# SAIC-MONTREAL/multimodal-dynamics

Measured on AMD Instinct MI355X. Metric: visuotactile samples/sec (train) + ELBO vs CPU ref, cnn-mvae 64x64 bs256 @1/2/4/8 GPU, higher is better.
Workload: dtype f32x3; 1 GPU; cnn-mvae visuotactile+pose 64x64, bs=256 per GPU, fp32 storage and results, GEMMs in the fp32x3 arithmetic (exact three-term bf16 split of the fp32 operands, six of nine products on the bf16 matrix cores, fp32 accumulate; error vs fp64 <= native fp32 MFMA), seq_modeling train step (7 subset ELBOs + backward + Adam), BASELINE configs[1]; global_batch=256, parallelism=dp1, bn=local, launch=hip_graph

## Files before the change

include/mmdyn_hip.h:

```cpp
#ifndef MMDYN_HIP_H
#define MMDYN_HIP_H

#include <stdint.h>

#ifdef __cplusplus
extern "C" {
#endif

#define MMDYN_OK 0
#define MMDYN_ERR_SHAPE (-1)
#define MMDYN_ERR_NULL (-2)
#define MMDYN_ERR_RANGE (-3)

#define MMDYN_ACT_NONE 0
#define MMDYN_ACT_SWISH 1
#define MMDYN_ACT_RELU 2

#define MMDYN_DENSE 0
#define MMDYN_CONV 1
#define MMDYN_TCONV_S2P1 2
#define MMDYN_IM2COL3 3

#define MMDYN_TCONV_S1P0 4

// ... 16 lines not shown
int mmdyn_igemm_slab_floats(int mode, int G, int Bg, int Hi, int Wi, int Cin, int Ho, int Wo, int N);

int mmdyn_igemm_nt_bf16(const float* A, const float* Bp, const float* bias, float* C, float* C_act,
                        float* stats, float* ws, int mode, int G, int Bg, int Hi, int Wi, int Cin,
                        int Ho, int Wo, int N, int ldc, int stride, int offset, int act, int splitk,
                        void* stream);
int mmdyn_igemm_nt_f16(const float* A, const float* Bp, const float* bias, float* C, float* C_act,
                       float* stats, float* ws, int mode, int G, int Bg, int Hi, int Wi, int Cin,
                       int Ho, int Wo, int N, int ldc, int stride, int offset, int act, int splitk,
                       void* stream);
int mmdyn_igemm_stat_tiles(int mode, int G, int Bg, int Hi, int Wi, int Cin, int Ho, int Wo, int N);
int mmdyn_igemm_stat_tiles_bf16(int mode, int G, int Bg, int Hi, int Wi, int Cin, int Ho, int Wo, int N);
int mmdyn_igemm_stat_tiles_mx(int mode, int G, int Bg, int Hi, int Wi, int Cin, int Ho, int Wo, int N, int flags);
int mmdyn_igemm_slab_floats_mx(int mode, int G, int Bg, int Hi, int Wi, int Cin, int Ho, int Wo, int N, int flags);
int mmdyn_igemm_nt_grouped(const void* A, const void* Bp, const float* bias, void* C, void* C_act, const void* u, int G,
                           int rows, int K, int N, int act, int flags, void* stream);
int mmdyn_splitk_reduce(const float* ws, const float* bias, float* C, float* C_act, int splitk,
                        int rows, int N, int act, void* stream);

int mmdyn_wgrad_tn(const float* D, const float* Gt, float* partial, int mode, int Bt, int Hr, int Wr,
                   int Cd, int Hi, int Wi, int Cg, int stride, int offset, int chunks, void* stream);
int mmdyn_wgrad_tn_bf16(const float* D, const float* Gt, float* partial, int mode, int Bt, int Hr, int Wr,
                        int Cd, int Hi, int Wi, int Cg, int stride, int offset, int chunks, void* stream);
int mmdyn_wgrad_tn_f16(const float* D, const float* Gt, float* partial, int mode, int Bt, int Hr, int Wr,
                       int Cd, int Hi, int Wi, int Cg, int stride, int offset, int chunks, void* stream);
int mmdyn_wgrad_tn_grouped(const void* D, const void* Gt, float* partial, int G, int rows, int Cd, int Cg, int chunks,
                           int flags, void* stream);
int mmdyn_wgrad_out3_bn(const void* y, const float* mean, const float* rstd, const float* gamma, const float* beta,
                        const float* Gt, float* partial, int G, int Bg, int Hr, int chunks, int y_b16, void* stream);
int mmdyn_wgrad_chunks(int mode, int rows, int Cd, int Cg);
int mmdyn_wgrad_chunks_mx(int mode, int rows, int Cd, int Cg, int flags);
int mmdyn_wgrad_reduce(const float* partial, float* canon, int chunks, int taps, int Cd, int Cg,
                       int cg_canon, int perm, float beta, void* stream);

int mmdyn_pack_conv_weight(const float* Wc, float* P, int d0, int d1, int swap, void* stream);
int mmdyn_repack2d(const float* in, float* out, int rows_in, int cols_in, int rows_out, int cols_out,
                   int mode, void* stream);

int mmdyn_repack2d_ld(const float* in, float* out, int rows_in, int cols_in, int rows_out, int cols_out,
                      int ld_out, int mode, void* stream);
int mmdyn_pack_conv_weight_b16(const float* Wc, void* P, int d0, int d1, int swap, int half, void* stream);
int mmdyn_repack2d_ld_b16(const float* in, void* out, int rows_in, int cols_in, int rows_out, int cols_out,
                          int ld_out, int mode, int half, void* stream);
typedef struct {
  const float* src;
  float* dst;
  int kind, rows_in, cols_in, rows_out, cols_out, ld_out;
  int dst_bf16;
} mmdyn_pack_entry;
int mmdyn_pack_plan(const mmdyn_pack_entry* plan_dev, int n, void* stream);

int mmdyn_im2col_nchw3(const float* x, float* col, int Bt, int H, int W, void* stream);
int mmdyn_col2im_k4(const float* col, float* out, int Bt, int Hi, int Wi, int Ho, int Wo, int C,
                    int ldcol, int stride, int pad, int tap_major, void* stream);

int mmdyn_tconv_out3_fwd(const float* a, const float* w, float* out, int Bt, int Hi, int Wi, void* stream);
int mmdyn_tconv_out3_bn_fwd(const void* y, const float* mean, const float* rstd, const float* gamma, const float* beta,
                            const float* w, float* out, int G, int Bg, int Hi, int Wi, int b16, void* stream);
int mmdyn_tconv_out3_bn_bce(const void* y, const float* mean, const float* rstd, const float* gamma, const float* beta,
                            const float* w, float* logits, int logits_group, const float* target, const float* mask,
                            int mask_channels, float* dlogit, double* loss_slots, double* unmasked_slots,
                            const int* slot_of_group, float grad_scale, int G, int Bg, int Hi, int Wi, int b16, void* stream);
int mmdyn_tconv_out3_bn_bce_rows(const void* y, const float* mean, const float* rstd, const float* gamma, const float* beta,
                                 const float* w, float* logits, int logits_group, const float* target, const float* mask,
                                 int mask_channels, double* loss_rows, double* unmasked_rows, const int* slot_of_group,
                                 int n_slots, int G, int Bg, int Hi, int Wi, int b16, void* stream);
// ... 200 lines not shown
```

multimodal-dynamics_amd/csrc/wgrad_geom.h:

```cpp
#pragma once
#include "common.h"

struct WgradGeom {
  int d_b16, g_b16;
  int f16;
  int mode;
  int rows;
  int Hr, Wr, Cd;
  int Hi, Wi, Cg;
  int rs, ro;
  int ntaps, chunks, rows_per_chunk;
  int groups;
  int x3;
  int pre;
};

#ifdef MMDYN_LAB
int mmdyn_wgrad_ws_try(const float* D, const float* Gt, float* partial, const WgradGeom& g, hipStream_t st);
#else
static inline int mmdyn_wgrad_ws_try(const float*, const float*, float*, const WgradGeom&, hipStream_t) { return 1; }
#endif

int mmdyn_wgrad_p3_try(const void* D, const void* Gt, float* partial, const WgradGeom& g, int Bt, hipStream_t st);
int mmdyn_wgrad_p3_chunks(int rows, int Cd, int Cg);
```

multimodal-dynamics_amd/csrc/wgrad_tn.hip:

```cpp
#include <stdlib.h>
#include "common.h"
#include "wgrad_geom.h"

namespace {


constexpr int RK = 32;

typedef __bf16 bf16x4 __attribute__((ext_vector_type(4)));
typedef short s16x4 __attribute__((ext_vector_type(4)));
typedef _Float16 f16x4 __attribute__((ext_vector_type(4)));
__device__ __forceinline__ f16x4 pack4_f16(float a, float b, float c, float d) {
  f16x4 r;
  r[0] = (_Float16)a; r[1] = (_Float16)b; r[2] = (_Float16)c; r[3] = (_Float16)d;
  return r;
}
__device__ __forceinline__ s16x4 pack4_bf16(float a, float b, float c, float d) {
  bf16x4 r;
  r[0] = (__bf16)a; r[1] = (__bf16)b; r[2] = (__bf16)c; r[3] = (__bf16)d;
  return __builtin_bit_cast(s16x4, r);
}

template <int BX> struct x3_ld { static constexpr int v = (BX == 32) ? 32 : BX + 32; };
template <int MODE, int BD, int BG, int WD, int WG, int WK, bool BF16, int ST, bool X3 = false, int PRE = 0>
__global__ __launch_bounds__(256) void wgrad_tn_kernel(const float* __restrict__ D,
                                                       const float* __restrict__ Gt,
                                                       float* __restrict__ partial, const WgradGeom g) {
  static_assert(!X3 || (!BF16 && ST == 0 && WK == 1 && MODE != MMDYN_IM2COL3), "the three-term split is a variant of the fp32 kernel");
  static_assert(PRE == 0 || X3, "operands that arrive split belong to the three-term split arithmetic");
  constexpr bool PD = (PRE & 1) != 0, PG = (PRE & 2) != 0;
  constexpr int DT = WD / 32, GT = WG / 32;
  constexpr int WAVES_G = BG / WG;
  constexpr int WAVES_DG = (BD / WD) * WAVES_G;
  static_assert(WAVES_DG * WK == 4, "4 waves per block");
  constexpr int KPW = (RK / 2) / WK;
  constexpr int DV = BD / 4, GV = BG / 4;
  constexpr int D_LOADS = (RK * DV) / 256, G_LOADS = (RK * GV) / 256;
  static_assert(D_LOADS >= 1 && G_LOADS >= 1, "tile too small for 256 threads");

  extern __shared__ __attribute__((aligned(16))) char smem[];
  float* Ds = reinterpret_cast<float*>(smem);
  float* Gs = Ds + RK * BD;
  constexpr int LDD = x3_ld<BD>::v, LDG = x3_ld<BG>::v;
  bf16_t* Ds16 = reinterpret_cast<bf16_t*>(smem);
  bf16_t* Gs16 = Ds16 + 3 * RK * LDD;

  const int tid = threadIdx.x, lane = tid & 63, wave = tid >> 6;
  const int wk = wave / WAVES_DG, wdg = wave % WAVES_DG;
  const int wd = wdg / WAVES_G, wg = wdg % WAVES_G;
  const int tiles_g = g.Cg / BG;
  const int td = blockIdx.x / tiles_g, tg = blockIdx.x - td * tiles_g;
  const int cd0 = td * BD, cg0 = tg * BG;
  const int tap = blockIdx.y;
  const int ngrp = g.groups > 1 ? g.groups : 1;
  const int zb = gridDim.z / ngrp;
  const int grp = blockIdx.z / zb, chunk = blockIdx.z - grp * zb;
  const int dh = (MODE == MMDYN_CONV) ? (tap >> 2) : 0;
  const int dw = (MODE == MMDYN_CONV) ? (tap & 3) : 0;
  const int HWr = g.Hr * g.Wr;

  const int row_begin = grp * g.rows + chunk * g.rows_per_chunk;
  const int row_end = min((grp + 1) * g.rows, row_begin + g.rows_per_chunk);

  const float inv_hw = 1.0f / (float)HWr, inv_w = 1.0f / (float)g.Wr;
  auto fdiv = [](int n, int d, float inv, int& q, int& r) {
    q = (int)((float)n * inv);
    r = n - q * d;
    if (r < 0) { q -= 1; r += d; }
    if (r >= d) { q += 1; r -= d; }
  };
  f32x4 rd[D_LOADS], rg[G_LOADS];
  constexpr int DV8 = BD / 8, GV8 = BG / 8;
  constexpr int D_LOADS8 = (RK * DV8) / 256, G_LOADS8 = (RK * GV8) / 256;
  static_assert(PRE == 0 || (D_LOADS8 >= 1 && G_LOADS8 >= 1), "plane granules: tile too small for 256 threads");
  u32x4 pd[PD ? D_LOADS8 : 1][3], pg[PG ? G_LOADS8 : 1][3];
  unsigned okd = 0, okg = 0;
  auto gload = [&](int r0) {
    if constexpr (PD) {
#pragma unroll
      for (int i = 0; i < D_LOADS8; ++i) {
        const int idx = tid + 256 * i;
        const int r = idx / DV8, v = idx - r * DV8;
        const int row = r0 + r;
        const bool ok = row < row_end;
        const bf16_t* b = reinterpret_cast<const bf16_t*>(D) + (size_t)(ok ? row : 0) * 3 * g.Cd + cd0 + v * 8;
#pragma unroll
        for (int p = 0; p < 3; ++p) pd[i][p] = *reinterpret_cast<const u32x4*>(b + p * g.Cd);
        okd = ok ? (okd | (1u << i)) : (okd & ~(1u << i));
      }
    } else
#pragma unroll
    for (int i = 0; i < D_LOADS; ++i) {
      const int idx = tid + 256 * i;
      const int r = idx / DV, v = idx - r * DV;
      const int row = r0 + r;
// ... 120 lines not shown
          uint2 hh, mm, ll;
          split3_bf16(x[0], x[1], hh.x, mm.x, ll.x);
          split3_bf16(x[2], x[3], hh.y, mm.y, ll.y);
          *reinterpret_cast<uint2*>(&Gs16[o]) = hh;
          *reinterpret_cast<uint2*>(&Gs16[RK * LDG + o]) = mm;
          *reinterpret_cast<uint2*>(&Gs16[2 * RK * LDG + o]) = ll;
        }
      }
      return;
    }
#pragma unroll
    for (int i = 0; i < D_LOADS; ++i)
      reinterpret_cast<f32x4*>(Ds)[tid + 256 * i] = ((okd >> i) & 1u) ? rd[i] : zero;
#pragma unroll
    for (int i = 0; i < G_LOADS; ++i) {
      const unsigned m = okg >> (4 * i);
      f32x4 v;
      v[0] = (m & 1u) ? rg[i][0] : 0.f;
      v[1] = (m & 2u) ? rg[i][1] : 0.f;
      v[2] = (m & 4u) ? rg[i][2] : 0.f;
      v[3] = (m & 8u) ? rg[i][3] : 0.f;
      reinterpret_cast<f32x4*>(Gs)[tid + 256 * i] = v;
    }
  };

  f32x16 acc[DT][GT];
#pragma unroll
  for (int a = 0; a < DT; ++a)
#pragma unroll
    for (int b = 0; b < GT; ++b)
#pragma unroll
      for (int e = 0; e < 16; ++e) acc[a][b][e] = 0.f;

  const int h = lane >> 5, cl = lane & 31;
  if (row_begin < row_end) {
    gload(row_begin);
    lds_store();
    __syncthreads();
    for (int r0 = row_begin; r0 < row_end; r0 += RK) {
      gload(r0 + RK);
      __builtin_amdgcn_sched_barrier(0);
      if constexpr (X3) {
        const int gq = lane >> 4, tq = (lane >> 2) & 3, tp = lane & 3;
        const int trow = 8 * (gq >> 1) + tq, tcol = 16 * (gq & 1) + 4 * tp;
        typedef __attribute__((address_space(3))) s16x4* lds_s16x4_p;
        typedef __bf16 xb16x8 __attribute__((ext_vector_type(8)));
        auto frag = [&](const bf16_t* tile, int ld, int col0, int k0) {
          const s16x4 lo = __builtin_amdgcn_ds_read_tr16_b64_v4i16((lds_s16x4_p)(&tile[(k0 + trow) * ld + col0 + tcol]));
          const s16x4 hi = __builtin_amdgcn_ds_read_tr16_b64_v4i16((lds_s16x4_p)(&tile[(k0 + trow + 4) * ld + col0 + tcol]));
          typedef short s16x8 __attribute__((ext_vector_type(8)));
          const s16x8 v = {lo[0], lo[1], lo[2], lo[3], hi[0], hi[1], hi[2], hi[3]};
          return __builtin_bit_cast(xb16x8, v);
        };
#pragma unroll
        for (int kc = 0; kc < 2; ++kc) {
          xb16x8 pa[3][DT], pb[3][GT];
#pragma unroll
          for (int p = 0; p < 3; ++p) {
#pragma unroll
            for (int a = 0; a < DT; ++a) pa[p][a] = frag(Ds16 + p * RK * LDD, LDD, wd * WD + a * 32, kc * 16);
#pragma unroll
            for (int b = 0; b < GT; ++b) pb[p][b] = frag(Gs16 + p * RK * LDG, LDG, wg * WG + b * 32, kc * 16);
          }
          constexpr int order[6][2] = {{0, 2}, {2, 0}, {1, 1}, {0, 1}, {1, 0}, {0, 0}};
#pragma unroll
          for (int t = 0; t < 6; ++t)
// ... 26 lines not shown
          } else {
          s16x4 pa[DT], pb[GT];
#pragma unroll
          for (int a = 0; a < DT; ++a) {
            const float* p = &Ds[(r8 + 4 * h) * BD + wd * WD + a * 32 + cl];
            pa[a] = pack4_bf16(p[0], p[BD], p[2 * BD], p[3 * BD]);
          }
#pragma unroll
          for (int b = 0; b < GT; ++b) {
            const float* p = &Gs[(r8 + 4 * h) * BG + wg * WG + b * 32 + cl];
            pb[b] = pack4_bf16(p[0], p[BG], p[2 * BG], p[3 * BG]);
          }
#pragma unroll
          for (int a = 0; a < DT; ++a)
#pragma unroll
            for (int b = 0; b < GT; ++b)
              acc[a][b] = __builtin_amdgcn_mfma_f32_32x32x8bf16_1k(pa[a], pb[b], acc[a][b], 0, 0, 0);
          }
        }
      } else
#pragma unroll
      for (int kk = wk * KPW; kk < (wk + 1) * KPW; ++kk) {
        float af[DT], bf[GT];
#pragma unroll
        for (int a = 0; a < DT; ++a) af[a] = Ds[(2 * kk + h) * BD + wd * WD + a * 32 + cl];
#pragma unroll
        for (int b = 0; b < GT; ++b) bf[b] = Gs[(2 * kk + h) * BG + wg * WG + b * 32 + cl];
#pragma unroll
        for (int a = 0; a < DT; ++a)
#pragma unroll
          for (int b = 0; b < GT; ++b)
            acc[a][b] = __builtin_amdgcn_mfma_f32_32x32x2f32(af[a], bf[b], acc[a][b], 0, 0, 0);
      }
      __builtin_amdgcn_sched_barrier(0);
      __syncthreads();
      lds_store();
      __syncthreads();
    }
  }

  float* out = partial + ((size_t)(((chunk * WK + wk) * ngrp + grp) * g.ntaps + tap) * g.Cd) * g.Cg;
#pragma unroll
  for (int a = 0; a < DT; ++a)
#pragma unroll
    for (int e = 0; e < 16; ++e) {
      const int cd = cd0 + wd * WD + a * 32 + (e & 3) + 8 * (e >> 2) + 4 * h;
#pragma unroll
      for (int b = 0; b < GT; ++b) {
        const int cg = cg0 + wg * WG + b * 32 + cl;
        out[(size_t)cd * g.Cg + cg] = acc[a][b][e];
      }
    }
}

typedef __bf16 wb16x8 __attribute__((ext_vector_type(8)));
typedef _Float16 wf16x8 __attribute__((ext_vector_type(8)));
typedef float wacc16_t __attribute__((ext_vector_type(16)));
template <bool H16> __device__ __forceinline__ wacc16_t mfma16(wb16x8 a, wb16x8 b, wacc16_t c) {
  if constexpr (H16)
    return __builtin_amdgcn_mfma_f32_32x32x16_f16(__builtin_bit_cast(wf16x8, a), __builtin_bit_cast(wf16x8, b), c, 0, 0, 0);
  else
    return __builtin_amdgcn_mfma_f32_32x32x16_bf16(a, b, c, 0, 0, 0);
}
template <int BX> struct b16_ld { static constexpr int v = (BX == 32) ? 32 : BX + 32; };

template <int MODE, int BD, int BG, int WD, int WG, int WK, bool H16>
__global__ __launch_bounds__(256) __attribute__((amdgpu_waves_per_eu(1, 4))) void wgrad_b16_kernel(const bf16_t* __restrict__ D, const bf16_t* __restrict__ Gt,
                                                        float* __restrict__ partial, const WgradGeom g) {
  constexpr int DT = WD / 32, GT = WG / 32;
  constexpr int WAVES_G = BG / WG;
  constexpr int WAVES_DG = (BD / WD) * WAVES_G;
  static_assert(WAVES_DG * WK == 4 && (WK == 1 || WK == 2), "4 waves per block, at most two of them share a tile");
  constexpr int LDD = b16_ld<BD>::v, LDG = b16_ld<BG>::v;
// ... 724 lines not shown
        else if (g.pre == 2) WGRAD_X3(2);
        else if (g.pre == 1) WGRAD_X3(1);
        else WGRAD_X3(0);
#undef WGRAD_X3
      } else {
        if (g.pre) return MMDYN_ERR_SHAPE;
        if (smem > 65536)
          if (int e = x3_dense_opt_in.ensure((const void*)wgrad_tn_kernel<MMDYN_DENSE, BD, BG, WD, WG, WK, false, 0, true>, (int)smem)) return e;
        hipLaunchKernelGGL((wgrad_tn_kernel<MMDYN_DENSE, BD, BG, WD, WG, WK, false, 0, true>), grid, dim3(256), smem, st, D, Gt, partial, g);
      }
      MMDYN_LAUNCH_CHECK();
    }
  }
#define WGRAD_LAUNCH(M, BF, ST_)                                                                                      \
  hipLaunchKernelGGL((wgrad_tn_kernel<M, BD, BG, WD, WG, WK, BF, ST_>), grid, dim3(256), smem, st, D, Gt, partial, g)
#define WGRAD_MODE(M)                                                  \
  do {                                                                 \
    if (bf16 && g.f16 && g.d_b16 && g.g_b16) WGRAD_LAUNCH(M, true, 5); \
    else if (bf16 && g.f16 && g.d_b16) WGRAD_LAUNCH(M, true, 6);       \
    else if (bf16 && g.f16 && g.g_b16) WGRAD_LAUNCH(M, true, 7);       \
    else if (bf16 && g.d_b16 && g.g_b16) WGRAD_LAUNCH(M, true, 1);     \
    else if (bf16 && g.d_b16) WGRAD_LAUNCH(M, true, 2);                \
    else if (bf16 && g.g_b16) WGRAD_LAUNCH(M, true, 3);                \
    else if (bf16 && g.f16) WGRAD_LAUNCH(M, true, 4);                  \
    else if (bf16) WGRAD_LAUNCH(M, true, 0);                           \
    else WGRAD_LAUNCH(M, false, 0);                                    \
  } while (0)
  if (g.mode == MMDYN_CONV) WGRAD_MODE(MMDYN_CONV);
  else if (g.mode == MMDYN_DENSE) WGRAD_MODE(MMDYN_DENSE);
  else if constexpr (BG == 64) WGRAD_MODE(MMDYN_IM2COL3);
  else return MMDYN_ERR_SHAPE;
#undef WGRAD_MODE
#undef WGRAD_LAUNCH
  MMDYN_LAUNCH_CHECK();
}

}

static bool tile_128x64() {
  const char* e = lab_env("MMDYN_WGRAD_128x64");
  return !(e && e[0] == '0');
}

static bool p3_enabled() {
  const char* e = lab_env("MMDYN_WGRAD_P3");
  return !(e && e[0] == '0');
}

static int wgrad_entry(const float* D, const float* Gt, float* partial, int mode, int Bt, int Hr,
                       int Wr, int Cd, int Hi, int Wi, int Cg, int stride, int offset, int chunks,
                       void* stream, bool bf16, int storage_flags = 0, int groups = 1) {
  if (!D || !Gt || !partial) return MMDYN_ERR_NULL;
  if (groups < 1 || (groups > 1 && mode != MMDYN_DENSE)) return MMDYN_ERR_SHAPE;
  if (Cd % 32 || Cg % 32 || Cd <= 0 || Cg <= 0 || chunks < 4 || chunks % 4) return MMDYN_ERR_SHAPE;
  if (mode != MMDYN_DENSE && mode != MMDYN_CONV && mode != MMDYN_IM2COL3) return MMDYN_ERR_SHAPE;
  if (mode == MMDYN_IM2COL3 && (Cg != 64 || Hi != 2 * Hr || Wi != 2 * Wr)) return MMDYN_ERR_SHAPE;
  WgradGeom g{};
  bool x3 = (storage_flags & 128) != 0;
  const int pre = (storage_flags >> 8) & 3;
  storage_flags &= ~(128 | 256 | 512);
  if (x3 && (bf16 || storage_flags)) return MMDYN_ERR_SHAPE;
  if (pre && (!x3 || mode != MMDYN_CONV || groups > 1)) return MMDYN_ERR_SHAPE;
  if (const char* e = lab_env("MMDYN_X3_WGRAD")) x3 = e[0] == '1';
  g.x3 = x3 && !bf16;
  g.pre = pre;
  if (pre && !g.x3) return MMDYN_ERR_SHAPE;
// ... 108 lines not shown
  const int taps = (mode == MMDYN_CONV) ? 16 : 1;
  long tiles = (long)(Cd / bd) * (Cg / bg) * taps;
  if (mode == MMDYN_CONV && !(Cd % 64 == 0 && Cg % 64 == 0)) {
    tiles = (long)(Cd / bd) * (Cg / bg) * 4;
    wk = 1;
  }
  long target = 768;
  if (x3 && mode != MMDYN_IM2COL3) {
    target = 512;
  }
  if (const char* ov = lab_env("MMDYN_WGRAD_BLOCKS")) target = atol(ov);
  if (mode == MMDYN_IM2COL3) {
    tiles = 1;
    wk = 1;
  }
  long z = target / tiles;
  const long zmax = rows / 128;
  if (z > zmax) z = zmax;
  if (z < 1) z = 1;
  long chunks = z * wk;
  chunks = (chunks + 3) / 4 * 4;
  return (int)chunks;
}

extern "C" int mmdyn_wgrad_chunks(int mode, int rows, int Cd, int Cg) { return wgrad_chunks_impl(mode, rows, Cd, Cg, false); }
extern "C" int mmdyn_wgrad_chunks_mx(int mode, int rows, int Cd, int Cg, int flags) {
  if ((flags & 896) == 896 && !(flags & 1) && mode == MMDYN_CONV && p3_enabled()) {
    const int c = mmdyn_wgrad_p3_chunks(rows, Cd, Cg);
    if (c > 0) return c;
  }
  return wgrad_chunks_impl(mode, rows, Cd, Cg, (flags & 6) == 6, (flags & 128) != 0 && !(flags & 1));
}

extern "C" int mmdyn_wgrad_reduce(const float* partial, float* canon, int chunks, int taps, int Cd, int Cg,
                                  int cg_canon, int perm, float beta, void* stream) {
  if (!partial || !canon) return MMDYN_ERR_NULL;
  if (cg_canon > Cg || cg_canon <= 0) return MMDYN_ERR_SHAPE;
  if (perm == 1 && (Cg % 256 || Cg / 256 != 25)) return MMDYN_ERR_SHAPE;
  if (perm == 2 && (Cd % 256 || Cd / 256 != 25)) return MMDYN_ERR_SHAPE;
  int64_t slab = (int64_t)taps * Cd * Cg;
  if (chunks <= 64 && slab >= 65536) {
    hipLaunchKernelGGL(wgrad_reduce_vec_kernel, dim3(ew_grid(slab >> 2)), dim3(256), 0, (hipStream_t)stream, partial,
                       canon, chunks, taps, Cd, Cg, cg_canon, perm, beta);
    MMDYN_LAUNCH_CHECK();
  }
  int64_t ntiles = (slab + 31) / 32;
  int grid = (int)(ntiles < 8192 ? ntiles : 8192);
  hipLaunchKernelGGL(wgrad_reduce_kernel, dim3(grid), dim3(256), 0, (hipStream_t)stream, partial, canon, chunks,
                     taps, Cd, Cg, cg_canon, perm, beta);
  MMDYN_LAUNCH_CHECK();
}
```

multimodal-dynamics_amd/mmdyn_hip/_lib.py:

```python
import ctypes
import os

_HERE = os.path.dirname(os.path.abspath(__file__))
LIB_PATH = os.environ.get("MMDYN_HIP_LIB") or os.path.join(_HERE, "libmmdyn_hip.so")

_P, _I, _L, _F, _Q = ctypes.c_void_p, ctypes.c_int, ctypes.c_int64, ctypes.c_float, ctypes.c_uint64


class PassExperts(ctypes.Structure):
    _fields_ = [("mu", _P * 4), ("lv", _P * 4), ("dmu", _P * 4), ("dlv", _P * 4), ("ld", _I * 4), ("dz", _P * 3),
                ("zdst", _P * 3), ("zpl", _P * 3)]


class PackEntry(ctypes.Structure):
    _fields_ = [("src", _P), ("dst", _P), ("kind", _I), ("rows_in", _I), ("cols_in", _I), ("rows_out", _I),
                ("cols_out", _I), ("ld_out", _I), ("dst_bf16", _I)]


class FeedGroups(ctypes.Structure):
    _fields_ = [("recon", _P * 4), ("obs", _P * 4), ("out", _P * 4), ("row_len", _I * 4), ("logits", _I * 4), ("column", _I * 4)]


MAX_PASSES = 8
MAX_EXPERTS = 4
FEED_GROUPS = 4
ABI_VERSION = 6

_SIGNATURES = {
    "mmdyn_abi_version": "",
    "mmdyn_igemm_nt": "ppppppp" + "iiiiiiiiiiiiii" + "p",
    "mmdyn_igemm_nt_dgrad_bn": "ppppppppp" + "iiiiiiiiiiii" + "ppp",
    "mmdyn_igemm_nt_dgrad_act": "pppp" + "i" + "iiiiiiiiiii" + "i" + "ppp",
    "mmdyn_igemm_slab_floats": "iiiiiiiii",
    "mmdyn_igemm_nt_bf16": "ppppppp" + "iiiiiiiiiiiiii" + "p",
    "mmdyn_igemm_nt_f16": "ppppppp" + "iiiiiiiiiiiiii" + "p",
    "mmdyn_igemm_stat_tiles": "iiiiiiiii",
    "mmdyn_igemm_stat_tiles_bf16": "iiiiiiiii",
    "mmdyn_igemm_stat_tiles_mx": "iiiiiiiiii",
    "mmdyn_igemm_slab_floats_mx": "iiiiiiiiii",
    "mmdyn_igemm_nt_grouped": "pppppp" + "iiiiii" + "p",
    "mmdyn_splitk_reduce": "pppp" + "iiii" + "p",
    "mmdyn_wgrad_tn": "ppp" + "iiiiiiiiiii" + "p",
    "mmdyn_wgrad_tn_bf16": "ppp" + "iiiiiiiiiii" + "p",
    "mmdyn_wgrad_tn_f16": "ppp" + "iiiiiiiiiii" + "p",
    "mmdyn_wgrad_tn_grouped": "ppp" + "iiiiii" + "p",
    "mmdyn_wgrad_chunks": "iiii",
    "mmdyn_wgrad_chunks_mx": "iiiii",
    "mmdyn_wgrad_reduce": "pp" + "iiiiii" + "f" + "p",
    "mmdyn_pack_conv_weight": "pp" + "iii" + "p",
    "mmdyn_repack2d": "pp" + "iiiii" + "p",
    "mmdyn_repack2d_ld": "pp" + "iiiiii" + "p",
    "mmdyn_pack_conv_weight_b16": "pp" + "iiii" + "p",
    "mmdyn_repack2d_ld_b16": "pp" + "iiiiiii" + "p",
    "mmdyn_pack_plan": "p" + "i" + "p",
    "mmdyn_im2col_nchw3": "pp" + "iii" + "p",
    "mmdyn_col2im_k4": "pp" + "iiiiiiiiii" + "p",
    "mmdyn_tconv_out3_fwd": "ppp" + "iii" + "p",
    "mmdyn_tconv_out3_bn_fwd": "ppppppp" + "iiiii" + "p",
    "mmdyn_tconv_out3_bn_bce": "ppppppp" + "i" + "pp" + "i" + "pppp" + "f" + "iiiii" + "p",
    "mmdyn_wgrad_out3_bn": "ppppppp" + "iiiii" + "p",
    "mmdyn_colstats": "pp" + "iii" + "p",
    "mmdyn_colstats_tiles": "i",
    "mmdyn_bn_finalize": "ppppppp" + "iiii" + "ff" + "i" + "pp",
    "mmdyn_bn_swish_fwd": "pppppp" + "iii" + "p",
    "mmdyn_bn_swish_bwd_reduce": "ppppppp" + "iii" + "p",
    "mmdyn_bn_bwd_finalize": "ppppp" + "iii" + "f" + "pp",
    "mmdyn_bn_eval_stats": "pppp" + "ii" + "f" + "p",
    "mmdyn_bn_reduce_partials": "ppp" + "iii" + "p",
    "mmdyn_bn_finalize_sums": "pppppp" + "iii" + "ff" + "i" + "p",
    "mmdyn_bn_bwd_finalize_sums": "pppp" + "ii" + "ff" + "p",
    "mmdyn_bn_swish_bwd_apply": "pppppppp" + "iiii" + "p",
    "mmdyn_act_fwd": "pp" + "l" + "i" + "p",
    "mmdyn_act_bwd": "ppp" + "l" + "i" + "p",
    "mmdyn_dropout_expand": "ppp" + "iii" + "f" + "p",
    "mmdyn_dropout_reduce": "ppp" + "iii" + "f" + "pi" + "pp",
    "mmdyn_random_masks": "p" + "l" + "f" + "QQ" + "pp",
    "mmdyn_random_normal": "p" + "l" + "QQ" + "pp",
    "mmdyn_counter_add": "p" + "Q" + "p",
    "mmdyn_colsum": "ppp" + "iii" + "f" + "pp",
    "mmdyn_colsum_chunks": "i",
    "mmdyn_scale_dev": "ppp" + "l" + "p",
# ... 101 lines not shown
```

multimodal-dynamics_amd/mmdyn_hip/layers.py:

```python
import weakref

import torch

from . import ops
from .ops import ACT_NONE, ACT_SWISH, ACT_RELU, DENSE, CONV, TCONV_S2P1, IM2COL3, TCONV_S1P0
from .models.shapes import BN_EPS, BN_MOMENTUM, FEAT


def _new(like, *shape, dtype=torch.float32):
    if isinstance(like, ops.Planes):
        like = like.t
    return torch.empty(shape, device=like.device, dtype=dtype)


ACT_DTYPE = torch.float32
W_DTYPE = torch.float32


def _act(like, *shape):
    return torch.empty(shape, device=like.device, dtype=ACT_DTYPE)


def _cdiv(a, b):
    return (a + b - 1) // b
# ... 263 lines not shown
    return dy


def dgrad_bn_swish_backward(x, Wp, mode, G, Bg, Hi, Cin, Ho, N, stride, offset, y, mean, rstd, bn, dgamma, dbeta, planes_out=False,
                            eval_mode=False):
    rows_per_group = Bg * Ho * Ho
    if eval_mode:
        _eval_mode_check()
    if y.dtype == torch.float32 and mode != IM2COL3:
        x, Wp = split_operands(x, Wp, mode, G, Bg, Hi, Cin, Ho, N)
    if isinstance(x, ops.Planes):
        T = ops.B.igemm_stat_tiles(mode, G, Bg, Hi, Hi, Cin, Ho, Ho, N, planes=True)
    else:
        T = ops.B.igemm_stat_tiles(mode, G, Bg, Hi, Hi, Cin, Ho, Ho, N, all16=ops._is16(x) and ops._is16(Wp))
    du = torch.empty_like(y)
    partial = _new(y, G, T, 2, N)
    ops.B.igemm_nt_dgrad_bn(x, Wp, du, partial, y, mean, rstd, bn.gamma, bn.beta, mode, G, Bg, Hi, Hi, Cin, Ho, Ho, N,
                            stride, offset)
    if eval_mode:
        if dgamma is not None or dbeta is not None:
            _bn_eval_param_grads(y, partial, T, dgamma, dbeta, G, N)
        dy, dyp = _apply_out(y, planes_out)
        ops.backend_op("bn_eval_swish_bwd")(du, None, mean, rstd, bn.gamma, bn.beta, dy, None, G, rows_per_group, N, True, planes=dyp)
        return dy if dyp is None else dyp
    sums = _bn_backward_sums(y, partial, T, dgamma, dbeta, G, N)
    dy, dyp = _apply_out(y, planes_out)
    if dyp is not None:
        ops.B.bn_swish_bwd_apply(du, y, mean, rstd, bn.gamma, bn.beta, sums, None, G, rows_per_group, N, True, planes=dyp)
        return dyp
    ops.B.bn_swish_bwd_apply(du, y, mean, rstd, bn.gamma, bn.beta, sums, dy, G, rows_per_group, N, True)
    return dy


def wgrad(D, Gt, canon, mode, Bt, Hr, Cd, Hi, Cg, stride=1, offset=0, cg_canon=None, perm=0, defer=None):
    if defer is not None:
        defer.append((D, Gt, canon, mode, Bt, Hr, Cd, Hi, Cg, stride, offset, cg_canon, perm))
        return
    rows = Bt * Hr * Hr
    taps = 16 if mode == CONV else 1
    if isinstance(D, ops.Planes) or isinstance(Gt, ops.Planes):
        chunks = ops.B.wgrad_chunks(mode, rows, Cd, Cg, planes=(isinstance(D, ops.Planes), isinstance(Gt, ops.Planes)))
    else:
        chunks = ops.B.wgrad_chunks(mode, rows, Cd, Cg)
    partial = _new(D, chunks, taps, Cd, Cg)
    ops.B.wgrad_tn(D, Gt, partial, mode, Bt, Hr, Hr, Cd, Hi, Hi, Cg, stride, offset, chunks)
    ops.B.wgrad_reduce(partial, canon, chunks, taps, Cd, Cg, Cg if cg_canon is None else cg_canon, perm, 0.0)


def run_deferred_wgrads(queue):
    while queue:
        item = queue.pop(0)
        if item and callable(item[0]):
            item[0](*item[1:])
        else:
            wgrad(*item)


def bn_stats_only(y, partial, T, bn, G, rows_per_group, C, repeat=1):
    if partial is None:
        return _eval_stats(y, bn, G, C)
    return _bn_forward_stats(y, partial, T, bn, G, rows_per_group, C, repeat)


def fuses_last_bn(S):
    return S in (64, 128, 256)


def wgrad_out3_bn(y, mean, rstd, bn, dlogits, canon, G, Bg, Hr, defer=None):
    if defer is not None:
        defer.append((wgrad_out3_bn, y, mean, rstd, bn, dlogits, canon, G, Bg, Hr))
        return
    rows = G * Bg * Hr * Hr
# ... 579 lines not shown
        ops.B.repack2d(gb[:L], grads["linear_means.bias"], L, 1, L, 1, 0)
        ops.B.repack2d(gb[L:], grads["linear_log_var.bias"], L, 1, L, 1, 0)
    if not need_dx:
        return None
    dx, _ = dense(dout, c["pk"]["WhT"], None, rows, 2 * L, Kp)
    return dx if Kp == c["K0"] else crop_columns(dx, Kp, c["K0"])


def heads_group_buffers(Ps, like, w_dtype=None):
    L, K = Ps[0]["linear_means.weight"].shape
    Kp, G = _pad32(K), len(Ps)
    wd = W_DTYPE if w_dtype is None else w_dtype
    allb = {"Wh": torch.zeros(G, 2 * L, Kp, device=like.device, dtype=wd), "bh": torch.zeros(G, 2 * L, device=like.device),
            "WhT": torch.zeros(G, Kp, 2 * L, device=like.device, dtype=wd)}
    return allb, [{k: v[g] for k, v in allb.items()} for g in range(G)]


def heads_forward_grouped(hd_all, pk_all, G, rows):
    _, N, Kp = pk_all["Wh"].shape
    out = _new(hd_all, G * rows, N)
    ops.B.igemm_nt_grouped(hd_all, pk_all["Wh"], pk_all["bh"], out, None, None, G, rows, Kp, N, ACT_NONE)
    return out


def heads_backward_grouped(dout_all, pk_all, G, rows):
    _, N, Kp = pk_all["Wh"].shape
    dx = _new(dout_all, G * rows, Kp)
    ops.B.igemm_nt_grouped(dout_all, pk_all["WhT"], None, dx, None, None, G, rows, N, Kp, ACT_NONE)
    return dx


def heads_wgrad_grouped(hd_all, dout_all, pk_all, gW_all, gb, G, rows):
    _, N, Kp = pk_all["Wh"].shape
    chunks = ops.B.wgrad_chunks(DENSE, rows, N, Kp)
    partial = _new(hd_all, chunks, G, N, Kp)
    ops.B.wgrad_tn_grouped(dout_all, hd_all, partial, G, rows, N, Kp, chunks)
    ops.B.wgrad_reduce(partial, gW_all, chunks, 1, G * N, Kp, Kp, 0, 0.0)
    for g in range(G):
        ops.B.colsum(dout_all[g * rows:(g + 1) * rows], gb[g], rows, N, 0, 0.0)


HEAD_KEYS = ["linear_means.weight", "linear_means.bias", "linear_log_var.weight", "linear_log_var.bias"]
POSE_ENC_KEYS = ["fc_net.0.weight", "fc_net.0.bias", "fc_net.2.weight", "fc_net.2.bias"]
POSE_DEC_KEYS = ["deconv_net.0.weight", "deconv_net.0.bias", "deconv_net.2.weight", "deconv_net.2.bias",
                 "deconv_net.4.weight", "deconv_net.4.bias"]


def pose_encoder_trunk_forward(P, pose, out=None):
    _, h1 = linear_forward(pose, P["fc_net.0.weight"], P["fc_net.0.bias"], ACT_RELU)
    _, h2 = linear_forward(h1, P["fc_net.2.weight"], P["fc_net.2.bias"], ACT_NONE, out=out)
    return h2, {"x": pose, "h1": h1}


def pose_mlp_pack_specs(P, keys):
    out = []
    for k in keys:
        N, K = P[k].shape
        if K % 32 == 0 and N % 32 == 0:
            out.append(_spec(k + "T", P[k], 1, N, K, K, N, (K, N)))
    return out


def pose_encoder_trunk_backward(P, c, dh2, grads, packed=None):
    pk = packed or {}
    du1 = linear_backward(dh2, c["h1"], P["fc_net.2.weight"], grads["fc_net.2.weight"], grads["fc_net.2.bias"],
                          x_act=ACT_RELU, Wt=pk.get("fc_net.2.weightT"))
    linear_backward(du1, c["x"], P["fc_net.0.weight"], grads["fc_net.0.weight"], grads["fc_net.0.bias"],
                    need_dx=False)


# ... 16 lines not shown
```

multimodal-dynamics_amd/mmdyn_hip/ops.py:

```python
import ctypes

import os

import torch

from . import _lib
from ._lib import PassExperts, FeedGroups, MAX_PASSES, MAX_EXPERTS, FEED_GROUPS, check

ACT_NONE, ACT_SWISH, ACT_RELU = 0, 1, 2
DENSE, CONV, TCONV_S2P1, IM2COL3, TCONV_S1P0 = 0, 1, 2, 3, 4
ROW_GROUPS_MAX = 8


def _ptr(t, dtype=torch.float32):
    if t is None:
        return None
    if not t.is_cuda:
        raise RuntimeError("mmdyn_hip: the HIP path needs GPU tensors (got a CPU tensor); there is no CPU fallback")
    if t.dtype != dtype:
        raise TypeError(f"mmdyn_hip: expected {dtype}, got {t.dtype}")
    if not t.is_contiguous():
        raise ValueError("mmdyn_hip: tensor must be contiguous")
    return t.data_ptr()

# ... 322 lines not shown
        check(self.lib.mmdyn_splitk_reduce(_ptr(ws), _ptr(bias), _ptr(C), _ptr(C_act), splitk, rows, N, act,
                                           _stream()), "mmdyn_splitk_reduce")

    def wgrad_tn(self, D, Gt, partial, mode, Bt, Hr, Wr, Cd, Hi, Wi, Cg, stride, offset, chunks):
        if isinstance(D, Planes) or isinstance(Gt, Planes):
            if not self._x3() or mode != CONV:
                raise ValueError("mmdyn_hip: plane operands belong to the convolution-level weight gradients of the fp32x3 arithmetic")
            flags, ptrs = 128, []
            for k, (t, C) in enumerate(((D, Cd), (Gt, Cg))):
                if isinstance(t, Planes):
                    if t.C != C or not t.t.is_cuda or not t.t.is_contiguous():
                        raise ValueError("mmdyn_hip: wgrad_tn: plane operand of the wrong shape")
                    flags |= 256 << k
                    ptrs.append(t.t.data_ptr())
                else:
                    ptrs.append(_ptr(t))
            check(self.lib.mmdyn_wgrad_tn_mx(ptrs[0], ptrs[1], _ptr(partial), mode, Bt, Hr, Wr, Cd, Hi, Wi, Cg, stride, offset, chunks,
                                             flags, _stream()), "mmdyn_wgrad_tn_mx")
            return
        (pd, d16), (pg, g16) = _aptr(D), _aptr(Gt)
        if d16 or g16:
            check(self.lib.mmdyn_wgrad_tn_mx(pd, pg, _ptr(partial), mode, Bt, Hr, Wr, Cd, Hi, Wi, Cg, stride, offset, chunks,
                                             self._mx(d16, g16) | (2 if d16 else 0) | (4 if g16 else 0), _stream()),
                  "mmdyn_wgrad_tn_mx")
            return
        if self._x3():
            check(self.lib.mmdyn_wgrad_tn_mx(pd, pg, _ptr(partial), mode, Bt, Hr, Wr, Cd, Hi, Wi, Cg, stride, offset, chunks, 128,
                                             _stream()), "mmdyn_wgrad_tn_mx")
            return
        fn = {"fp32": self.lib.mmdyn_wgrad_tn, "fp16": self.lib.mmdyn_wgrad_tn_f16,
              "fp16s": self.lib.mmdyn_wgrad_tn_f16}.get(self.precision, self.lib.mmdyn_wgrad_tn_bf16)
        check(fn(pd, pg, _ptr(partial), mode, Bt, Hr, Wr, Cd, Hi, Wi, Cg, stride, offset, chunks,
                 _stream()), "mmdyn_wgrad_tn")

    def wgrad_reduce(self, partial, canon, chunks, taps, Cd, Cg, cg_canon, perm, beta):
        check(self.lib.mmdyn_wgrad_reduce(_ptr(partial), _ptr(canon), chunks, taps, Cd, Cg, cg_canon, perm,
                                          float(beta), _stream()), "mmdyn_wgrad_reduce")

    def pack_conv_weight(self, Wc, P, d0, d1, swap):
        pp, p16 = _aptr(P)
        if p16:
            check(self.lib.mmdyn_pack_conv_weight_b16(_ptr(Wc), pp, d0, d1, int(swap), _half(p16), _stream()),
                  "mmdyn_pack_conv_weight_b16")
            return
        check(self.lib.mmdyn_pack_conv_weight(_ptr(Wc), pp, d0, d1, int(swap), _stream()), "mmdyn_pack_conv_weight")

    def repack2d(self, src, dst, rows_in, cols_in, rows_out, cols_out, mode):
        if _is16(dst):
            return self.repack2d_ld(src, dst, rows_in, cols_in, rows_out, cols_out, cols_out, mode)
        check(self.lib.mmdyn_repack2d(_ptr(src), _ptr(dst), rows_in, cols_in, rows_out, cols_out, mode, _stream()),
              "mmdyn_repack2d")

    def repack2d_ld(self, src, dst, rows_in, cols_in, rows_out, cols_out, ld_out, mode):
        _, d16 = _aptr(dst)
        if d16:
            check(self.lib.mmdyn_repack2d_ld_b16(_ptr(src), dst.data_ptr(), rows_in, cols_in, rows_out, cols_out, ld_out, mode,
                                                 _half(d16), _stream()), "mmdyn_repack2d_ld_b16")
            return
        check(self.lib.mmdyn_repack2d_ld(_ptr(src), dst.data_ptr(), rows_in, cols_in, rows_out, cols_out, ld_out, mode,
                                         _stream()), "mmdyn_repack2d_ld")

    def concat_condition(self, x, cond, out, K, cd, bad_index=None):
        rows, width = out.shape
        if not x.is_cuda or x.dtype != torch.float32 or x.dim() != 2 or x.shape[0] != rows or x.shape[1] < K or \
                (x.stride(1) != 1 and x.shape[1] > 1) or (rows > 1 and x.stride(0) < K):
            raise ValueError("mmdyn_concat_condition: x must be fp32 GPU rows [rows][>= K] of unit element stride")
# ... 649 lines not shown
```

multimodal-dynamics_amd/mmdyn_hip/profiling.py:

```python
import collections

import torch

from . import ops

PAD_CYCLES = 100000
HOST_ONLY = {"igemm_stat_tiles", "colstats_tiles", "wgrad_chunks", "igemm_planes_served"}


def _canon(name, a):
    if name == "igemm_nt_dgrad_bn":
        A, Bp, C, stats, y, mean, rstd, gamma, beta, mode, G, Bg, Hi, Wi, Cin, Ho, Wo, N, stride, offset = a
        name, a = "igemm_nt", (A, Bp, y, C, None, stats, None, mode, G, Bg, Hi, Wi, Cin, Ho, Wo, N, N, stride, offset, 0, 1)
    if name == "igemm_nt_dgrad_act":
        A, Bp, C, u, act, mode, G, Bg, Hi, Wi, Cin, Ho, Wo, N, stride, offset = a
        name, a = "igemm_nt", (A, Bp, u, C, None, None, None, mode, G, Bg, Hi, Wi, Cin, Ho, Wo, N, N, stride, offset, 0, 1)
    if name == "igemm_nt_grouped":
        A, Bp, bias, C, C_act, u, G, rows, K, N, act = a
        name, a = "igemm_nt", (A, Bp, bias if u is None else u, C, C_act, None, None, ops.DENSE, G, rows, 1, 1, K, 1, 1, N, N, 1, 0, act, 1)
    if name == "wgrad_tn_grouped":
        D, Gt, partial, G, rows, Cd, Cg, chunks = a
        name, a = "wgrad_tn", (D, Gt, partial, ops.DENSE, G * rows, 1, 1, Cd, 1, 1, Cg, 1, 0, chunks)
    if name == "wgrad_out3_bn":
        y, mean, rstd, gamma, beta, Gt, partial, G, Bg, Hr, chunks = a
        return "conv3_wgrad", (y, Gt, partial, ops.IM2COL3, G * Bg, Hr, Hr, 32, 2 * Hr, 2 * Hr, 64, 1, 0, chunks)
    if name == "tconv_out3_bn_fwd":
        return "tconv_out3_fwd", a
    if name == "igemm_nt" and a[7] == ops.IM2COL3 and a[10] in (64, 128, 256) and \
            tuple(a[10:17]) == (a[10], a[10], 64, a[10] // 2, a[10] // 2, 32, 32):
        return "conv3_nt", a
    if name == "igemm_nt" and a[7] == ops.TCONV_S2P1 and tuple(a[10:16]) in ((16, 16, 64, 32, 32, 32), (32, 32, 32, 64, 64, 32),
                                                                            (64, 64, 32, 128, 128, 32)) and \
            getattr(ops.B, "precision", "fp32") == "fp32" and all(not torch.is_tensor(t) or t.dtype == torch.float32 for t in a[:4]):
        return "tconv_patch", a
    if name == "wgrad_tn" and a[3] == ops.IM2COL3 and a[8] in (64, 128, 256) and \
            tuple(a[5:11]) == (a[8] // 2, a[8] // 2, 32, a[8], a[8], 64):
        return "conv3_wgrad", a
    return name, a


def _flops(name, a):
    if name in ("igemm_nt", "conv3_nt", "tconv_patch"):
        (mode, G, Bg, Hi, Wi, Cin, Ho, Wo, N) = a[7:16]
        if mode == ops.DENSE:
            return 2.0 * G * Bg * Ho * Wo * N * Cin
        if mode == ops.CONV:
            return 2.0 * G * Bg * Ho * Wo * N * 16 * Cin
        if mode == ops.TCONV_S1P0:
            return 2.0 * G * Bg * Hi * Wi * N * 16 * Cin
        if mode == ops.IM2COL3:
            return 2.0 * G * Bg * Ho * Wo * N * 48
        return 2.0 * G * Bg * Ho * Wo * N * 4 * Cin
    if name in ("wgrad_tn", "conv3_wgrad"):
        (mode, Bt, Hr, Wr, Cd, Hi, Wi, Cg) = a[3:11]
        return 2.0 * Bt * Hr * Wr * Cd * Cg * (16 if mode == ops.CONV else 1)
# ... 22 lines not shown
        return self._inner.precision

    @precision.setter
    def precision(self, value):
        self._inner.precision = value

    @property
    def fp32_split(self):
        return getattr(self._inner, "fp32_split", False)

    @fp32_split.setter
    def fp32_split(self, value):
        self._inner.fp32_split = value

    def __getattr__(self, attr):
        fn = getattr(self._inner, attr)
        if attr in HOST_ONLY or not callable(fn):
            return fn

        def wrapped(*a, **k):
            s, e = torch.cuda.Event(enable_timing=True), torch.cuda.Event(enable_timing=True)
            torch.cuda._sleep(PAD_CYCLES)
            s.record()
            r = fn(*a, **k)
            e.record()
            name, ca = _canon(attr, a)
            sig = tuple(x for x in ca if isinstance(x, (int, bool))) if name in ("igemm_nt", "wgrad_tn", "conv3_nt", "conv3_wgrad", "tconv_patch") else ()
            if attr == "igemm_nt_dgrad_bn":
                sig = sig + ("bn_bwd_epilogue",)
            if attr == "igemm_nt_dgrad_act":
                sig = sig + ("act_bwd_epilogue",)
            if attr in ("igemm_nt_grouped", "wgrad_tn_grouped"):
                sig = sig + ("grouped",)
            self.records.append((name, _flops(name, ca), _bytes(ca), s, e, sig))
            return r
        return wrapped

    def summary(self):
        torch.cuda.synchronize()
        agg = collections.OrderedDict()
        self.by_shape = collections.OrderedDict()
        for name, fl, by, s, e, sig in self.records:
            if sig:
                d2 = self.by_shape.setdefault((name,) + sig, {"calls": 0, "ms": 0.0, "flops": 0.0})
                d2["calls"] += 1
                d2["ms"] += s.elapsed_time(e)
                d2["flops"] += fl
            d = agg.setdefault(name, {"calls": 0, "ms": 0.0, "flops": 0.0, "bytes": 0.0})
            d["calls"] += 1
            d["ms"] += s.elapsed_time(e)
            d["flops"] += fl
            d["bytes"] += by
        return agg


def profile_step(fn):
    timed = TimedBackend(ops.B)
    old = ops.set_backend(timed)
    try:
        fn()
    finally:
        ops.set_backend(old)
    out = timed.summary()
    profile_step.by_shape = timed.by_shape
    return out
```

Before: 52740 samples/s.

## Add direct-epilogue dense weight-gradient path that skips split-K partials and reduce

Adds a DIRECT variant of the weight-gradient TN kernel for dense layers. Each block walks the full row range, accumulating per-chunk sums into a running total to keep the split-K rounding order, and writes straight into the canonical gradient with the permutation and beta applied. Dense FC layers and the grouped heads use it whenever there are at least 256 output tiles and at most 4096 rows. This removes the partial buffer write/read and the separate reduce launch, but gives up split-K parallelism along rows and adds extra accumulator registers.

```diff
diff --git a/include/mmdyn_hip.h b/include/mmdyn_hip.h
--- a/include/mmdyn_hip.h
+++ b/include/mmdyn_hip.h
@@ -72,6 +72,9 @@
 int mmdyn_wgrad_chunks_mx(int mode, int rows, int Cd, int Cg, int flags);
 int mmdyn_wgrad_reduce(const float* partial, float* canon, int chunks, int taps, int Cd, int Cg,
                        int cg_canon, int perm, float beta, void* stream);
+int mmdyn_wgrad_direct_served(int rows, int Cd, int Cg, int G, int flags);
+int mmdyn_wgrad_direct(const void* D, const void* Gt, float* canon, int G, int rows, int Cd, int Cg, int cg_canon, int perm,
+                       float beta, int flags, void* stream);
 
 int mmdyn_pack_conv_weight(const float* Wc, float* P, int d0, int d1, int swap, void* stream);
 int mmdyn_repack2d(const float* in, float* out, int rows_in, int cols_in, int rows_out, int cols_out,
diff --git a/multimodal-dynamics_amd/csrc/wgrad_geom.h b/multimodal-dynamics_amd/csrc/wgrad_geom.h
--- a/multimodal-dynamics_amd/csrc/wgrad_geom.h
+++ b/multimodal-dynamics_amd/csrc/wgrad_geom.h
@@ -13,6 +13,8 @@
   int groups;
   int x3;
   int pre;
+  int cg_canon, perm;
+  float beta;
 };
 
 #ifdef MMDYN_LAB
diff --git a/multimodal-dynamics_amd/csrc/wgrad_tn.hip b/multimodal-dynamics_amd/csrc/wgrad_tn.hip
--- a/multimodal-dynamics_amd/csrc/wgrad_tn.hip
+++ b/multimodal-dynamics_amd/csrc/wgrad_tn.hip
@@ -22,12 +22,13 @@
 }
 
 template <int BX> struct x3_ld { static constexpr int v = (BX == 32) ? 32 : BX + 32; };
-template <int MODE, int BD, int BG, int WD, int WG, int WK, bool BF16, int ST, bool X3 = false, int PRE = 0>
+template <int MODE, int BD, int BG, int WD, int WG, int WK, bool BF16, int ST, bool X3 = false, int PRE = 0, bool DIRECT = false>
 __global__ __launch_bounds__(256) void wgrad_tn_kernel(const float* __restrict__ D,
                                                        const float* __restrict__ Gt,
                                                        float* __restrict__ partial, const WgradGeom g) {
   static_assert(!X3 || (!BF16 && ST == 0 && WK == 1 && MODE != MMDYN_IM2COL3), "the three-term split is a variant of the fp32 kernel");
   static_assert(PRE == 0 || X3, "operands that arrive split belong to the three-term split arithmetic");
+  static_assert(!DIRECT || (MODE == MMDYN_DENSE && WK == 1 && !BF16 && PRE == 0), "the direct epilogue: uncut DENSE launches in fp32 / the split");
   constexpr bool PD = (PRE & 1) != 0, PG = (PRE & 2) != 0;
   constexpr int DT = WD / 32, GT = WG / 32;
   constexpr int WAVES_G = BG / WG;
@@ -59,8 +60,8 @@
   const int dw = (MODE == MMDYN_CONV) ? (tap & 3) : 0;
   const int HWr = g.Hr * g.Wr;
 
-  const int row_begin = grp * g.rows + chunk * g.rows_per_chunk;
-  const int row_end = min((grp + 1) * g.rows, row_begin + g.rows_per_chunk);
+  const int row_begin = grp * g.rows + (DIRECT ? 0 : chunk * g.rows_per_chunk);
+  const int row_end = DIRECT ? (grp + 1) * g.rows : min((grp + 1) * g.rows, row_begin + g.rows_per_chunk);
 
   const float inv_hw = 1.0f / (float)HWr, inv_w = 1.0f / (float)g.Wr;
   auto fdiv = [](int n, int d, float inv, int& q, int& r) {
@@ -247,6 +248,16 @@
 #pragma unroll
       for (int e = 0; e < 16; ++e) acc[a][b][e] = 0.f;
 
+  f32x16 tot[DIRECT ? DT : 1][DIRECT ? GT : 1];
+  int ksteps = 0;
+  if constexpr (DIRECT) {
+#pragma unroll
+    for (int a = 0; a < DT; ++a)
+#pragma unroll
+      for (int b = 0; b < GT; ++b)
+#pragma unroll
+        for (int e = 0; e < 16; ++e) tot[a][b][e] = 0.f;
+  }
   const int h = lane >> 5, cl = lane & 31;
   if (row_begin < row_end) {
     gload(row_begin);
@@ -339,6 +350,19 @@
           for (int b = 0; b < GT; ++b)
             acc[a][b] = __builtin_amdgcn_mfma_f32_32x32x2f32(af[a], bf[b], acc[a][b], 0, 0, 0);
       }
+      if constexpr (DIRECT) {
+        if (++ksteps == g.rows_per_chunk / RK) {
+          ksteps = 0;
+#pragma unroll
+          for (int a = 0; a < DT; ++a)
+#pragma unroll
+            for (int b = 0; b < GT; ++b) {
+              tot[a][b] += acc[a][b];
+#pragma unroll
+              for (int e = 0; e < 16; ++e) acc[a][b][e] = 0.f;
+            }
+        }
+      }
       __builtin_amdgcn_sched_barrier(0);
       __syncthreads();
       lds_store();
@@ -346,6 +370,29 @@
     }
   }
 
+  if constexpr (DIRECT) {
+#pragma unroll
+    for (int a = 0; a < DT; ++a)
+#pragma unroll
+      for (int b = 0; b < GT; ++b) acc[a][b] = tot[a][b] + acc[a][b];
+    float* canon = partial + (size_t)grp * g.Cd * g.cg_canon;
+#pragma unroll
+    for (int a = 0; a < DT; ++a)
+#pragma unroll
+      for (int e = 0; e < 16; ++e) {
+        const int cd = cd0 + wd * WD + a * 32 + (e & 3) + 8 * (e >> 2) + 4 * h;
+        const int orow = (g.perm == 2) ? (cd & 255) * 25 + (cd >> 8) : cd;
+#pragma unroll
+        for (int b = 0; b < GT; ++b) {
+          const int cg = cg0 + wg * WG + b * 32 + cl;
+          if (cg >= g.cg_canon) continue;
+          const int ocol = (g.perm == 1) ? (cg & 255) * 25 + (cg >> 8) : cg;
+          float* o = canon + (size_t)orow * g.cg_canon + ocol;
+          *o = (g.beta != 0.f) ? (g.beta * *o + acc[a][b][e]) : acc[a][b][e];
+        }
+      }
+    return;
+  }
   float* out = partial + ((size_t)(((chunk * WK + wk) * ngrp + grp) * g.ntaps + tap) * g.Cd) * g.Cg;
 #pragma unroll
   for (int a = 0; a < DT; ++a)
@@ -1136,6 +1183,21 @@
   else return MMDYN_ERR_SHAPE;
 #undef WGRAD_MODE
 #undef WGRAD_LAUNCH
+  MMDYN_LAUNCH_CHECK();
+}
+
+template <int BD, int BG, int WD, int WG>
+static int launch_direct(const float* D, const float* Gt, float* canon, WgradGeom g, hipStream_t st) {
+  g.rows_per_chunk = ceil_div(ceil_div(g.rows, g.chunks), RK) * RK;
+  dim3 grid((g.Cd / BD) * (g.Cg / BG), 1, g.groups > 1 ? g.groups : 1);
+  if (g.x3) {
+    constexpr size_t smem = (size_t)3 * RK * (x3_ld<BD>::v + x3_ld<BG>::v) * 2;
+    static_assert(smem <= 65536, "no LDS opt-in on this path");
+    hipLaunchKernelGGL((wgrad_tn_kernel<MMDYN_DENSE, BD, BG, WD, WG, 1, false, 0, true, 0, true>), grid, dim3(256), smem, st, D, Gt, canon, g);
+  } else {
+    constexpr size_t smem = (size_t)RK * (BD + BG) * sizeof(float);
+    hipLaunchKernelGGL((wgrad_tn_kernel<MMDYN_DENSE, BD, BG, WD, WG, 1, false, 0, false, 0, true>), grid, dim3(256), smem, st, D, Gt, canon, g);
+  }
   MMDYN_LAUNCH_CHECK();
 }
 
@@ -1310,6 +1372,50 @@
   return wgrad_chunks_impl(mode, rows, Cd, Cg, (flags & 6) == 6, (flags & 128) != 0 && !(flags & 1));
 }
 
+static constexpr int DIRECT_MIN_TILES = 256;
+static constexpr int DIRECT_MAX_ROWS = 4096;
+static bool direct_flags_ok(int flags) { return flags == 0 || flags == 128; }
+
+extern "C" int mmdyn_wgrad_direct_served(int rows, int Cd, int Cg, int G, int flags) {
+  if (!direct_flags_ok(flags) || rows <= 0 || G < 1 || Cd <= 0 || Cg <= 0 || Cd % 64 || Cg % 64) return 0;
+  if (rows > DIRECT_MAX_ROWS) return 0;
+  return (long)(Cd / 64) * (Cg / 64) * G >= DIRECT_MIN_TILES ? 1 : 0;
+}
+
+extern "C" int mmdyn_wgrad_direct(const void* D, const void* Gt, float* canon, int G, int rows, int Cd, int Cg, int cg_canon,
+                                  int perm, float beta, int flags, void* stream) {
+  if (!D || !Gt || !canon) return MMDYN_ERR_NULL;
+  if (!direct_flags_ok(flags) || G < 1 || rows <= 0 || Cd <= 0 || Cg <= 0 || Cd % 64 || Cg % 64) return MMDYN_ERR_SHAPE;
+  if (cg_canon > Cg || cg_canon <= 0 || perm < 0 || perm > 2 || (perm && G > 1)) return MMDYN_ERR_SHAPE;
+  if (perm == 1 && (Cg != 6400 || cg_canon != Cg)) return MMDYN_ERR_SHAPE;
+  if (perm == 2 && Cd != 6400) return MMDYN_ERR_SHAPE;
+  if ((int64_t)G * rows * Cd >= (1LL << 31) || (int64_t)G * rows * Cg >= (1LL << 31) || (int64_t)Cd * Cg >= (1LL << 31)) return MMDYN_ERR_RANGE;
+  WgradGeom g{};
+  bool x3 = flags == 128;
+  if (const char* e = lab_env("MMDYN_X3_WGRAD")) x3 = e[0] == '1';
+  g.x3 = x3;
+  g.mode = MMDYN_DENSE;
+  g.groups = G;
+  g.rows = rows;
+  g.Hr = g.Wr = g.Hi = g.Wi = 1;
+  g.Cd = Cd;
+  g.Cg = Cg;
+  g.rs = 1;
+  g.ntaps = 1;
+  g.cg_canon = cg_canon;
+  g.perm = perm;
+  g.beta = beta;
+  g.chunks = wgrad_chunks_impl(MMDYN_DENSE, rows, Cd, Cg, false, flags == 128);
+  if (g.chunks < 1) return MMDYN_ERR_SHAPE;
+  const float* d = (const float*)D;
+  const float* gt = (const float*)Gt;
+#ifdef MMDYN_LAB
+  if (const char* e = getenv("MMDYN_WGRAD_DIRECT_TILE"))
+    if (e[0] == '1' && Cd % 128 == 0) return launch_direct<128, 64, 64, 32>(d, gt, canon, g, (hipStream_t)stream);
+#endif
+  return launch_direct<64, 64, 32, 32>(d, gt, canon, g, (hipStream_t)stream);
+}
+
 extern "C" int mmdyn_wgrad_reduce(const float* partial, float* canon, int chunks, int taps, int Cd, int Cg,
                                   int cg_canon, int perm, float beta, void* stream) {
   if (!partial || !canon) return MMDYN_ERR_NULL;
diff --git a/multimodal-dynamics_amd/mmdyn_hip/_lib.py b/multimodal-dynamics_amd/mmdyn_hip/_lib.py
--- a/multimodal-dynamics_amd/mmdyn_hip/_lib.py
+++ b/multimodal-dynamics_amd/mmdyn_hip/_lib.py
@@ -47,6 +47,8 @@
     "mmdyn_wgrad_chunks": "iiii",
     "mmdyn_wgrad_chunks_mx": "iiiii",
     "mmdyn_wgrad_reduce": "pp" + "iiiiii" + "f" + "p",
+    "mmdyn_wgrad_direct_served": "iiiii",
+    "mmdyn_wgrad_direct": "ppp" + "iiiiii" + "f" + "i" + "p",
     "mmdyn_pack_conv_weight": "pp" + "iii" + "p",
     "mmdyn_repack2d": "pp" + "iiiii" + "p",
     "mmdyn_repack2d_ld": "pp" + "iiiiii" + "p",
diff --git a/multimodal-dynamics_amd/mmdyn_hip/layers.py b/multimodal-dynamics_amd/mmdyn_hip/layers.py
--- a/multimodal-dynamics_amd/mmdyn_hip/layers.py
+++ b/multimodal-dynamics_amd/mmdyn_hip/layers.py
@@ -319,12 +319,26 @@
     return dy
 
 
+FC_WGRAD_DIRECT = True
+
+
+def fc_wgrad_direct(D, Gt, rows, Cd, Cg, G=1):
+    direct = getattr(ops.B, "wgrad_direct", None) if FC_WGRAD_DIRECT else None
+    if direct is None or not (torch.is_tensor(D) and torch.is_tensor(Gt) and D.dtype == Gt.dtype == torch.float32):
+        return None
+    return direct if ops.B.wgrad_direct_served(rows, Cd, Cg, G) else None
+
+
 def wgrad(D, Gt, canon, mode, Bt, Hr, Cd, Hi, Cg, stride=1, offset=0, cg_canon=None, perm=0, defer=None):
     if defer is not None:
         defer.append((D, Gt, canon, mode, Bt, Hr, Cd, Hi, Cg, stride, offset, cg_canon, perm))
         return
     rows = Bt * Hr * Hr
     taps = 16 if mode == CONV else 1
+    direct = fc_wgrad_direct(D, Gt, rows, Cd, Cg) if mode == DENSE else None
+    if direct is not None:
+        direct(D, Gt, canon, 1, rows, Cd, Cg, Cg if cg_canon is None else cg_canon, perm, 0.0)
+        return
     if isinstance(D, ops.Planes) or isinstance(Gt, ops.Planes):
         chunks = ops.B.wgrad_chunks(mode, rows, Cd, Cg, planes=(isinstance(D, ops.Planes), isinstance(Gt, ops.Planes)))
     else:
@@ -970,10 +984,14 @@
 
 def heads_wgrad_grouped(hd_all, dout_all, pk_all, gW_all, gb, G, rows):
     _, N, Kp = pk_all["Wh"].shape
-    chunks = ops.B.wgrad_chunks(DENSE, rows, N, Kp)
-    partial = _new(hd_all, chunks, G, N, Kp)
-    ops.B.wgrad_tn_grouped(dout_all, hd_all, partial, G, rows, N, Kp, chunks)
-    ops.B.wgrad_reduce(partial, gW_all, chunks, 1, G * N, Kp, Kp, 0, 0.0)
+    direct = fc_wgrad_direct(dout_all, hd_all, rows, N, Kp, G)
+    if direct is not None:
+        direct(dout_all, hd_all, gW_all, G, rows, N, Kp, Kp, 0, 0.0)
+    else:
+        chunks = ops.B.wgrad_chunks(DENSE, rows, N, Kp)
+        partial = _new(hd_all, chunks, G, N, Kp)
+        ops.B.wgrad_tn_grouped(dout_all, hd_all, partial, G, rows, N, Kp, chunks)
+        ops.B.wgrad_reduce(partial, gW_all, chunks, 1, G * N, Kp, Kp, 0, 0.0)
     for g in range(G):
         ops.B.colsum(dout_all[g * rows:(g + 1) * rows], gb[g], rows, N, 0, 0.0)
 
diff --git a/multimodal-dynamics_amd/mmdyn_hip/ops.py b/multimodal-dynamics_amd/mmdyn_hip/ops.py
--- a/multimodal-dynamics_amd/mmdyn_hip/ops.py
+++ b/multimodal-dynamics_amd/mmdyn_hip/ops.py
@@ -378,6 +378,20 @@
               "fp16s": self.lib.mmdyn_wgrad_tn_f16}.get(self.precision, self.lib.mmdyn_wgrad_tn_bf16)
         check(fn(pd, pg, _ptr(partial), mode, Bt, Hr, Wr, Cd, Hi, Wi, Cg, stride, offset, chunks,
                  _stream()), "mmdyn_wgrad_tn")
+
+    def _direct_flags(self):
+        return self._x3() if self.precision == "fp32" else None
+
+    def wgrad_direct_served(self, rows, Cd, Cg, G=1):
+        flags = self._direct_flags()
+        return flags is not None and self.lib.mmdyn_wgrad_direct_served(rows, Cd, Cg, G, flags) == 1
+
+    def wgrad_direct(self, D, Gt, canon, G, rows, Cd, Cg, cg_canon, perm, beta):
+        flags = self._direct_flags()
+        if flags is None:
+            raise ValueError(f"mmdyn_hip: wgrad_direct serves fp32 operands only (precision {self.precision!r})")
+        check(self.lib.mmdyn_wgrad_direct(_ptr(D), _ptr(Gt), _ptr(canon), G, rows, Cd, Cg, cg_canon, perm, float(beta), flags,
+                                          _stream()), "mmdyn_wgrad_direct")
 
     def wgrad_reduce(self, partial, canon, chunks, taps, Cd, Cg, cg_canon, perm, beta):
         check(self.lib.mmdyn_wgrad_reduce(_ptr(partial), _ptr(canon), chunks, taps, Cd, Cg, cg_canon, perm,
diff --git a/multimodal-dynamics_amd/mmdyn_hip/profiling.py b/multimodal-dynamics_amd/mmdyn_hip/profiling.py
--- a/multimodal-dynamics_amd/mmdyn_hip/profiling.py
+++ b/multimodal-dynamics_amd/mmdyn_hip/profiling.py
@@ -5,7 +5,7 @@
 from . import ops
 
 PAD_CYCLES = 100000
-HOST_ONLY = {"igemm_stat_tiles", "colstats_tiles", "wgrad_chunks", "igemm_planes_served"}
+HOST_ONLY = {"igemm_stat_tiles", "colstats_tiles", "wgrad_chunks", "igemm_planes_served", "wgrad_direct_served"}
 
 
 def _canon(name, a):
@@ -21,6 +21,9 @@
     if name == "wgrad_tn_grouped":
         D, Gt, partial, G, rows, Cd, Cg, chunks = a
         name, a = "wgrad_tn", (D, Gt, partial, ops.DENSE, G * rows, 1, 1, Cd, 1, 1, Cg, 1, 0, chunks)
+    if name == "wgrad_direct":
+        D, Gt, canon, G, rows, Cd, Cg, cg_canon, perm, beta = a
+        name, a = "wgrad_tn", (D, Gt, canon, ops.DENSE, G * rows, 1, 1, Cd, 1, 1, Cg, 1, 0, 1)
     if name == "wgrad_out3_bn":
         y, mean, rstd, gamma, beta, Gt, partial, G, Bg, Hr, chunks = a
         return "conv3_wgrad", (y, Gt, partial, ops.IM2COL3, G * Bg, Hr, Hr, 32, 2 * Hr, 2 * Hr, 64, 1, 0, chunks)
@@ -109,6 +112,8 @@
                 sig = sig + ("act_bwd_epilogue",)
             if attr in ("igemm_nt_grouped", "wgrad_tn_grouped"):
                 sig = sig + ("grouped",)
+            if attr == "wgrad_direct":
+                sig = sig + ("direct",)
             self.records.append((name, _flops(name, ca), _bytes(ca), s, e, sig))
             return r
         return wrapped
```

Result: no change. 53190 samples/s (median of 6 runs) (+0.9%).
